# sbyrnes321/metalens

Hardware: AMD Instinct MI355X
Metric: aperture x far-field pair-evals/sec (higher is better)
Workload: dtype f64; 1 GPU; 1 mm dia NA=0.5 lens, lambda=580 nm, 4096x4096 aperture window at pitch lambda/2.2 -> 512x512 far-field directions (bins of the aperture FFT lattice x 1), fp64, on-axis x-dipole at the focus; aperture=4096, farfield=512, rings=197, centre_cells=1219855, orders=survey, pmc_key=gpus=1,aperture=4096,farfield=512,precision=f64,method=auto,zoom=1,pols=1, pmc_stale=True

## Files before the change

metalens_amd/csrc/common.h:

```cpp
#pragma once

#include <hip/hip_runtime.h>

#include <algorithm>
#include <cstdarg>
#include <cstdlib>
#include <cstdint>
#include <cstdio>
#include <cstring>
#include <string>
#include <vector>

#include "metalens_hip.h"

namespace ml {

void set_error(const char *fmt, ...);

#define ML_HIP(call)                                                                      \
    do {                                                                                  \
        hipError_t e_ = (call);                                                           \
        if (e_ != hipSuccess) {                                                           \
            ml::set_error("%s failed: %s (%s:%d)", #call, hipGetErrorString(e_), __FILE__, \
                          __LINE__);                                                      \
// ... 364 lines not shown

namespace ml {

void prof_begin(ml_ctx *ctx, int kernel, hipEvent_t *a, hipEvent_t *b, hipStream_t stream = nullptr);
void prof_end(ml_ctx *ctx, int kernel, hipEvent_t a, hipEvent_t b, hipStream_t stream = nullptr);
int prof_harvest(ml_ctx *ctx);

struct ProfScope {
    ml_ctx *ctx;
    int kernel;
    hipStream_t stream;
    hipEvent_t a = nullptr, b = nullptr;
    ProfScope(ml_ctx *c, int k, hipStream_t s = nullptr) : ctx(c), kernel(k), stream(s) {
        prof_begin(ctx, kernel, &a, &b, stream);
    }
    ~ProfScope() { prof_end(ctx, kernel, a, b, stream); }
};

int zgemm(hipStream_t stream, int M, int N, int K, const double *alpha, const double *A,
          int64_t lda, int64_t strideA, const double *B, int64_t ldb, int64_t strideB, double *C,
          int64_t ldc, int64_t strideC, int batch, int accumulate);
int zcoldot(hipStream_t stream, int n_fields, int rows, int cols, const double *alpha4,
            const double *TX, int64_t ldtx, int j0, const double *G, double *out, int accumulate);
struct FoldIO {
    int in_slabs = 1;
    int64_t in_slab_stride = 0;
    int out_t_rows = 0;
    const double *out_E = nullptr;
};
int zfold_stage1(hipStream_t stream, int M, int ny, const double *A, int64_t lda, const double *Cm,
                 const double *Sm, const double *R4, int T, int S, const double *E,
                 const double *D, double *C, int64_t ldc, int my, const int *row_first = nullptr,
                 int nxl = 1, int ksplit = 1, int64_t split_stride = 0, bool f32 = false,
                 FoldIO io = FoldIO());
int zfold_splits(int T, int ksplit);
struct ZfftCall {
    int N_eff, n_valid, M, j0, pad1, pad2;
    int jstep = 1;
    const double *in;
    int64_t in_s1, in_s2, in_es;
    int in_rb, a0, h0, a1, h1;
    const int *row_first;
    int rf_mod;
    int sub_s = 1, sub_i = 0;
    double *out;
    int64_t out_s1, out_s2, out_es;
    int out_rb;
    const double *tw1, *wk, *pj;
    const int *kbin;
    double alpha[4];
    int alpha_rb, rows, accumulate;
    int passes = 0;
    int second = 0;
};
int zfft_split(int N_eff);
bool zfft_commensurate(int n, double step, long double kappa, const double *u, int M,
                       long double tol, int *N_eff, int *j0, int *jstep);
int zfft_build_tables(hipStream_t stream, double *tw1, double *wk, double *pj, int *kbin, int M,
                      int j0, int N_eff, int c, int jstep = 1);
void zfft_choose_pads(int N_eff, int M, int j0, int *pad1, int *pad2, int jstep = 1);
int zfft_run_interleaved(hipStream_t stream, const ZfftCall &c, int s, int64_t sub_off, int stuff);
int zfft_build_interleave_tables(hipStream_t stream, double *wk, double *pj, int *kbin, int M, int j0, int Nsub,
                                 int N, int c, int first, int block, int jstep = 1);
int zfft_run(hipStream_t stream, const ZfftCall &c);
void comm_release(ml_ctx *ctx);
int fields_unmodulate(ml_ctx *ctx);
int flush_unfold(ml_ctx *ctx);
int comm_allreduce_sum(ml_ctx *ctx, double *buf, size_t count, hipStream_t stream);
int comm_reduce_scatter_sum(ml_ctx *ctx, double *buf, size_t chunk, hipStream_t stream);
int comm_allgather(ml_ctx *ctx, double *buf, size_t chunk, hipStream_t stream);
int comm_join(ml_ctx *ctx, bool host);

int nearfield_launch(ml_ctx *ctx, const ml_nearfield_params *p, int n, int nx, int ny);
int power_flush(ml_ctx *ctx);
bool plan_cache_disabled();
constexpr int POWER_GROUPS = 32;
__device__ __forceinline__ void sum_partials_group(const double *partial, int n, double *groups,
                                                   int g, int tid) {
    __shared__ double s_part[256];
    const int lo = (int)((long long)n * g / POWER_GROUPS), hi = (int)((long long)n * (g + 1) / POWER_GROUPS);
    double acc = 0.0;
    for (int k = lo + tid; k < hi; k += 256) acc += partial[k];
    __syncthreads();
    s_part[tid] = acc;
    __syncthreads();
    for (int w = 128; w > 0; w >>= 1) {
        if (tid < w) s_part[tid] += s_part[tid + w];
        __syncthreads();
    }
    if (tid == 0) groups[g] = s_part[0];
}

}
```

metalens_amd/csrc/farfield.hip:

```cpp
#include <algorithm>
#include <cmath>
#include <cstdlib>
#include <cstring>
#include <vector>

#include <cfloat>

#include "common.h"

namespace ml {

#define ML_TWO_PI_HI 6.283185307179586232e+00
#define ML_TWO_PI_LO 2.449293598294706414e-16

__global__ __launch_bounds__(256) void twiddle_kernel(double2 *out, int rows, int cols,
                                                      int sample_major, int center, double s_hi,
                                                      double s_lo, const double *u) {
    const int c = blockIdx.x * 256 + threadIdx.x;
    const int r = blockIdx.y;
    if (c >= cols) return;
    const int sample = sample_major ? r : c;
    const int dir = sample_major ? c : r;
    const double kk = (double)(sample - center);
    const double uu = u[dir];
    const double p_hi = kk * s_hi;
    const double p_lo = fma(kk, s_hi, -p_hi) + kk * s_lo;
    const double q_hi = p_hi * uu;
    const double q_lo = fma(p_hi, uu, -q_hi) + p_lo * uu;
    const double f = (q_hi - rint(q_hi)) + q_lo;
    const double a_hi = f * ML_TWO_PI_HI;
    const double ang = a_hi + (fma(f, ML_TWO_PI_HI, -a_hi) + f * ML_TWO_PI_LO);
    double sn, cs;
    sincos(ang, &sn, &cs);
    out[(size_t)r * cols + c] = make_double2(cs, -sn);
}

constexpr int MAX_PHASE_JOBS = 6;
struct PhaseJob {
    double2 *out;
    double *outc, *outs;
    int rows, cols, sample_major, block0;
    double coord0, coord_step, s_hi, s_lo;
    const double *u_hi, *u_lo;
};
struct PhaseBatch {
    PhaseJob job[MAX_PHASE_JOBS];
    int n, blocks;
};

__global__ __launch_bounds__(256) void phase_batch_kernel(const PhaseBatch b) {
    int j = 0;
    for (int k = 1; k < b.n; ++k)
        if ((int)blockIdx.x >= b.job[k].block0) j = k;
    const PhaseJob &q = b.job[j];
    const int per_row = (q.cols + 255) / 256;
    const int local = blockIdx.x - q.block0;
    const int r = local / per_row, c = (local % per_row) * 256 + threadIdx.x;
    if (c >= q.cols) return;
    const int sample = q.sample_major ? r : c;
    const int dir = q.sample_major ? c : r;
    const double kk = q.coord0 + q.coord_step * (double)sample;
// ... 591 lines not shown
    pl.wavelength = wavelength;
    pl.n_glass = n_glass;
    pl.method = method;
    ML_TRY(upload_if_changed(ctx, pl.ux, pl.h_ux, ux, mx));
    ML_TRY(upload_if_changed(ctx, pl.uy, pl.h_uy, uy, my));
    ML_TRY(pl.tw_x.reserve((size_t)mx * nx_total * 2 * sizeof(double)));
    const size_t out_elems = pair_list ? (size_t)mx : (size_t)mx * my;
    ML_TRY(pl.vectors.reserve(4 * out_elems * 2 * sizeof(double)));
    ML_TRY(pl.power.reserve(out_elems * sizeof(double)));
    ML_TRY(pl.amplitudes.reserve(2 * 2 * out_elems * 2 * sizeof(double)));
    pl.fft_y.ok = pl.fft_x.ok = false;
    if (method != ML_METHOD_GEMM && !pair_list) {
        ML_TRY(plan_fft_axis(ctx, pl.fft_y, ny, dyp, uy, my));
        ML_TRY(plan_fft_axis(ctx, pl.fft_x, nx_total, dxp, ux, mx));
    }
    pl.fold = false;
    if (!pl.fft_y.ok) ML_TRY(plan_fold(ctx, uy));
    if (!pl.fold && !pl.fft_y.ok) {
        ML_TRY(pl.tw_y.reserve((size_t)ny * my * 2 * sizeof(double)));
        ML_TRY(launch_twiddle(ctx, pl.tw_y.as<double>(), ny, my, 1, ny, dyp, wavelength, n_glass,
                              pl.uy.as<double>()));
    }
    pl.tw_x_ready = false;
    ML_TRY(plan_fold2(ctx, ux));
    pl.ready = true;
    return ML_OK;
}

static int interleave_stuff(int n_sub) {
    for (int z = 1; z <= 8; z <<= 1)
        if ((n_sub * z) % 256 == 0) return z;
    return 0;
}

static int interleave_block(const FarfieldPlan &pl, int n_ranks) {
    if (!pl.ready || pl.pair_list || !pl.fft_x.ok || n_ranks < 2) return 0;
    const int N = pl.fft_x.N_eff;
    for (int s = 8; s >= 1; s >>= 1) {
        if (N % (s * n_ranks) != 0 || pl.nx_total % (s * n_ranks) != 0) continue;
        const int stuff = interleave_stuff(N / (s * n_ranks));
        if (!stuff) continue;
        const int r3 = N / (s * n_ranks) * stuff / 256;
        if (r3 >= 1 && r3 <= 32 && r3 * s <= 32) return s;
    }
    return 0;
}

struct Shard {
    int kind = 0;
    int row0 = 0;
    int block = 0, n_ranks = 1, rank = 0;
};

static int transform_impl(ml_ctx *ctx, const Shard &sh, int accumulate) {
    ML_REQUIRE(ctx, "ctx is NULL");
    const int row0 = sh.row0, mirrored = sh.kind == 1;
    FarfieldPlan &pl = ctx->plan;
    if (!pl.ready) {
        set_error("ml_farfield_plan has not been called");
        return ML_ESTATE;
    }
    if (ctx->nx == 0) {
        set_error("no resident field set");
        return ML_ESTATE;
    }
    ML_REQUIRE(ctx->ny == pl.ny, "resident fields have ny=%d but the plan has ny=%d", ctx->ny,
               pl.ny);
    if (sh.kind == 2) {
        ML_REQUIRE(sh.block >= 1 && sh.block == interleave_block(pl, sh.n_ranks),
                   "interleaved shard: block %d is not what ml_farfield_interleave_block gives for %d ranks "
                   "on this plan (%d)", sh.block, sh.n_ranks, interleave_block(pl, sh.n_ranks));
        ML_REQUIRE(sh.rank >= 0 && sh.rank < sh.n_ranks && ctx->nx == pl.nx_total / sh.n_ranks,
                   "interleaved shard: rank %d of %d with %d resident rows of %d", sh.rank, sh.n_ranks,
                   ctx->nx, pl.nx_total);
    } else if (mirrored) {
        ML_REQUIRE(ctx->nx % 2 == 0 && row0 >= 0 && 2 * row0 + ctx->nx <= pl.nx_total,
                   "mirrored shard: %d resident rows starting at %d do not form row pairs of a "
                   "%d-row aperture", ctx->nx, row0, pl.nx_total);
        ML_REQUIRE(!pl.pair_list, "mirrored shards are for tensor grids");
    } else {
        ML_REQUIRE(row0 >= 0 && row0 + ctx->nx <= pl.nx_total,
                   "rows [%d, %d) fall outside the planned aperture of %d rows", row0,
                   row0 + ctx->nx, pl.nx_total);
    }
    ML_REQUIRE(!accumulate || pl.have_vectors, "accumulate requested but nothing to add to");
    ML_HIP(hipSetDevice(ctx->device));
    if (accumulate)
        ML_TRY(flush_unfold(ctx));
    else
        pl.unfold_pending = false;
    const int nxl = ctx->nx, ny = pl.ny, mx = pl.mx, my = pl.my;
    pl.stage1_splits = 1;
    int want_split1 = 1;
    if (pl.fold) {
        const long t128 = (long)((4 * nxl + 31) / 32) * ((pl.fold_S + 127) / 128);
        const long t64 = (long)((4 * nxl + 31) / 32) * ((pl.fold_S + 63) / 64);
        if (t128 >= 480)
            want_split1 = 1;
        else if (2 * t128 >= 480)
            want_split1 = 2;
        else
            want_split1 = (int)std::min<long>(8, std::max<long>(1, (640 + t64 - 1) / std::max<long>(t64, 1)));
        static const int forced_split = diag_int("ML_STAGE1_SPLIT", 0);
        if (forced_split > 0) want_split1 = forced_split;
        pl.stage1_splits = zfold_splits(pl.fold_T, want_split1);
    }
#ifndef ML_STAGE1_TRANSPOSED
#define ML_STAGE1_TRANSPOSED 1
#endif
    const bool g_transposed = ML_STAGE1_TRANSPOSED && pl.fft_y.ok && pl.fft_x.ok && !pl.pair_list &&
                              pl.fft_y.split == 1 && pl.fft_x.split == 1 && sh.kind != 2 &&
                              (pl.method == ML_METHOD_FFT_STREAMED ||
                               (size_t)nxl * ny * 8 + (size_t)4 * nxl * my * 16 > (size_t)96 << 20);
    static const int g_skew = diag_int("ML_G_SKEW", 8);
    const int64_t g_ld = nxl + g_skew;
    static const bool pieces_off = [] { const char *e = getenv("METALENS_HIP_PIECES"); return e && e[0] == '0'; }();
    const size_t g_bytes = g_transposed ? (size_t)4 * my * g_ld * 2 * sizeof(double)
                                        : (size_t)pl.stage1_splits * 4 * nxl * my * 2 * sizeof(double);
    const bool pieced = g_transposed && nxl <= 8192 && !pieces_off && pl.stage1_pieces.reserve(g_bytes) == ML_OK;
    if (!pieced) ML_TRY(pl.stage1.reserve(g_bytes));
    double *const g_buf = pieced ? pl.stage1_pieces.as<double>() : pl.stage1.as<double>();
    static const long fold2_min_tiles = diag_int("ML_FOLD2_MIN_TILES", 32);
    const bool whole = (row0 == 0 && nxl == pl.nx_total);
    const bool fold2_pays = (long)((4 * my + 31) / 32) * ((pl.fold2_S + 63) / 64) >= fold2_min_tiles;
    const bool fft1 = pl.fft_y.ok, fft2 = pl.fft_x.ok && !pl.pair_list;
    int trim_lo = 0, trim_hi = nxl;
    if (fft1 && fft2 && !mirrored && ctx->row_first_valid && (int)ctx->h_x_pts.size() == nxl &&
        (int)ctx->h_y_pts.size() == ny && ctx->r_outer > 0) {
        if (ctx->trim_key[0] != ctx->grid_serial || ctx->trim_key[1] != ctx->layout_serial) {
            double ymin = INFINITY;
            for (double y : ctx->h_y_pts) ymin = std::min(ymin, std::fabs(y));
            int lo = nxl, hi = 0;
            for (int i = 0; i < nxl; ++i) {
                const double x = ctx->h_x_pts[i];
                if (!(std::sqrt(x * x + ymin * ymin) > ctx->r_outer)) {
                    lo = std::min(lo, i);
                    hi = i + 1;
                }
            }
            if (lo >= hi) lo = 0, hi = std::min(nxl, 1);
            ctx->trim_rows[0] = lo;
            ctx->trim_rows[1] = hi;
            ctx->trim_key[0] = ctx->grid_serial;
            ctx->trim_key[1] = ctx->layout_serial;
        }
        static const bool no_trim = diag_int("ML_NO_ROW_TRIM", 0) != 0;
        if (!no_trim) {
            trim_lo = ctx->trim_rows[0];
            trim_hi = ctx->trim_rows[1];
        }
    }
    const int nxt = trim_hi - trim_lo;
    const bool use_fold2 = !fft2 && !pl.pair_list && pl.fold2 && fold2_pays && (mirrored || whole) && sh.kind != 2;
    static const bool no_direct = diag_int("ML_NO_GT_DIRECT", 0) != 0;
    const bool gt_direct = pl.fold && use_fold2 && !no_direct;
    FoldIO io1;
    int want_split2 = 1;
    if (gt_direct) {
        ML_TRY(stage2_tables(ctx, row0, mirrored, &want_split2));
        io1.out_t_rows = nxl;
        io1.out_E = pl.fold2_has_E ? pl.fold2_E.as<double>() : nullptr;
    }
    bool fields_premodulated = false;
    if (ctx->fields_premod_serial >= 0) {
        if (ctx->fields_premod_serial != pl.serial || !pl.fold) {
            set_error("the resident fields carry the input modulation of an earlier far-field plan "
                      "(ml_nearfield_premodulate): synthesise them again after ml_farfield_plan");
            return ML_ESTATE;
        }
        fields_premodulated = true;
    }
    const double one[4] = {1.0, 1.0, 1.0, 1.0};
    auto launch_fft1 = [&]() -> int {
        ZfftCall c;
        const int split1 = pl.fft_y.split;
        c.passes = pl.fft_y.passes;
        c.N_eff = pl.fft_y.N_eff / split1;
        c.n_valid = ny;
        c.M = my;
        c.j0 = pl.fft_y.j0;
        c.jstep = pl.fft_y.jstep;
        c.pad1 = pl.fft_y.pad1;
        c.pad2 = pl.fft_y.pad2;
        c.in = ctx->set_ptr() + (size_t)trim_lo * ny * 2;
        c.rows = 4 * nxt;
        c.in_rb = nxt;
        c.in_s1 = (int64_t)nxl * ny;
        c.in_s2 = ny;
        c.in_es = 1;
        c.a0 = 0;
        c.h0 = ny;
        c.a1 = c.h1 = 0;
        c.row_first = ctx->row_first_valid ? ctx->row_first.as<int>() + trim_lo : nullptr;
        c.rf_mod = nxt;
        c.out = g_buf + (size_t)trim_lo * my * 2;
        c.out_rb = nxt;
        c.out_s1 = (int64_t)nxl * my;
        c.out_s2 = my;
        c.out_es = 1;
        if (g_transposed) {
            c.out = g_buf + (size_t)trim_lo * 2;
            c.out_rb = nxt;
            c.out_s1 = (int64_t)my * g_ld;
            c.out_s2 = 1;
            c.out_es = g_ld;
        }
        c.tw1 = pl.fft_tw1.as<double>();
        c.wk = pl.fft_y.wk.as<double>();
        c.pj = pl.fft_y.pj.as<double>();
        c.kbin = pl.fft_y.kbin.as<int>();
        for (int k = 0; k < 4; ++k) c.alpha[k] = 1.0;
        c.alpha_rb = c.rows;
        c.accumulate = 0;
        if (split1 > 1) {
            for (int i = 0; i < split1; ++i) {
                c.sub_s = split1;
                c.sub_i = i;
                c.pj = pl.fft_y.pj.as<double>() + (size_t)i * my * 2;
                c.accumulate = i > 0;
                ML_TRY(zfft_run(ctx->stream, c));
            }
        } else {
            ML_TRY(zfft_run(ctx->stream, c));
        }
        return ML_OK;
    };
    {
        ProfScope scope(ctx, ML_K_ZGEMM_STAGE1);
        if (fft1) {
            ML_TRY(launch_fft1());
        } else if (pl.fold)
            ML_TRY(zfold_stage1(ctx->stream, 4 * nxl, ny, ctx->set_ptr(), ny,
                                pl.fold_cm.as<double>(), pl.fold_sm.as<double>(),
                                pl.fold_r4.as<double>(), pl.fold_T,
                                pl.fold_S,
                                pl.fold_has_E && !fields_premodulated ? pl.fold_E.as<double>() : nullptr,
                                pl.fold_D.as<double>(), g_buf, my, my,
                                ctx->row_first_valid ? ctx->row_first.as<int>() : nullptr, nxl,
                                want_split1, (int64_t)4 * nxl * my, ctx->gemm_f32 != 0, io1));
        else
            ML_TRY(zgemm(ctx->stream, 4 * nxl, my, ny, one, ctx->set_ptr(), ny, 0,
                         pl.tw_y.as<double>(), my, 0, g_buf, my, 0, 1, 0));
    }
    const double dA = pl.dxp * pl.dyp;
    const double alpha[4] = {-dA, dA, dA, -dA};
    auto collapse_stage1 = [&]() -> int {
        if (pl.stage1_splits > 1) {
            const size_t n = (size_t)4 * nxl * my;
            hipLaunchKernelGGL(zsum_slabs_kernel, dim3((unsigned)((n + 255) / 256)), dim3(256), 0,
                               ctx->stream, reinterpret_cast<double2 *>(g_buf), n, pl.stage1_splits);
            ML_HIP(hipGetLastError());
            pl.stage1_splits = 1;
        }
        return ML_OK;
    };
    if (sh.kind == 2) {
        ProfScope scope(ctx, ML_K_ZGEMM_STAGE2);
        ML_TRY(collapse_stage1());
// ... 14 lines not shown
        {
            ZfftCall c;
            c.N_eff = Nsub;
            c.n_valid = n_have;
            c.M = mx;
            c.j0 = pl.fft_x.j0;
            c.jstep = pl.fft_x.jstep;
            c.pad1 = pl.il_pad1;
            c.pad2 = pl.il_pad2;
            c.in = g_buf;
            c.rows = 4 * my;
            c.in_rb = my;
            c.in_s1 = (int64_t)nxl * my;
            c.in_s2 = 1;
            c.in_es = (int64_t)s * my;
            c.a0 = trim_lo;
            c.h0 = nxt;
            c.a1 = c.h1 = 0;
            c.row_first = nullptr;
            c.rf_mod = 1;
            c.out = pl.vectors.as<double>() + (size_t)3 * mx * my * 2;
            c.out_rb = my;
            c.out_s1 = -(int64_t)mx * my;
            c.out_s2 = 1;
            c.out_es = my;
            c.tw1 = pl.fft_tw1.as<double>();
            c.wk = pl.il_wk.as<double>();
            c.pj = pl.il_pj.as<double>();
            c.kbin = pl.il_kbin.as<int>();
            for (int k = 0; k < 4; ++k) c.alpha[k] = alpha[k];
            c.alpha_rb = my;
            c.accumulate = accumulate;
            ML_TRY(zfft_run_interleaved(ctx->stream, c, s, my, stuff));
        }
    } else if (fft2) {
        ProfScope scope(ctx, ML_K_ZGEMM_STAGE2);
        ML_TRY(collapse_stage1());
        ZfftCall c;
        const int split2 = pl.fft_x.split;
        c.passes = pl.fft_x.passes;
        c.N_eff = pl.fft_x.N_eff / split2;
        c.n_valid = pl.nx_total;
        c.M = mx;
        c.j0 = pl.fft_x.j0;
        c.jstep = pl.fft_x.jstep;
        c.pad1 = pl.fft_x.pad1;
        c.pad2 = pl.fft_x.pad2;
        c.in = g_buf;
        c.rows = 4 * my;
        c.in_rb = my;
        c.in_s1 = (int64_t)nxl * my;
        c.in_s2 = 1;
        c.in_es = my;
        if (g_transposed) {
            c.in_s1 = (int64_t)my * g_ld;
            c.in_s2 = g_ld;
            c.in_es = 1;
            c.second = 1;
        }
        if (mirrored) {
            c.a0 = row0;
            c.h0 = nxl / 2;
            c.a1 = pl.nx_total - row0 - nxl / 2;
            c.h1 = nxl / 2;
        } else {
            c.a0 = row0 + trim_lo;
            c.h0 = nxt;
            c.a1 = c.h1 = 0;
            c.in = g_buf + (size_t)trim_lo * c.in_es * 2;
        }
        c.row_first = nullptr;
        c.rf_mod = 1;
        c.out = pl.vectors.as<double>() + (size_t)3 * mx * my * 2;
        c.out_rb = my;
        c.out_s1 = -(int64_t)mx * my;
        c.out_s2 = 1;
        c.out_es = my;
        c.tw1 = pl.fft_tw1.as<double>();
        c.wk = pl.fft_x.wk.as<double>();
        c.pj = pl.fft_x.pj.as<double>();
        c.kbin = pl.fft_x.kbin.as<int>();
        for (int k = 0; k < 4; ++k) c.alpha[k] = alpha[k];
        c.alpha_rb = my;
        for (int i = 0; i < split2; ++i) {
            c.sub_s = split2;
            c.sub_i = i;
            c.pj = pl.fft_x.pj.as<double>() + (size_t)i * mx * 2;
            c.accumulate = i > 0 ? 1 : accumulate;
            ML_TRY(zfft_run(ctx->stream, c));
        }
    } else if (use_fold2) {
        ProfScope scope(ctx, ML_K_ZGEMM_STAGE2);
        ML_TRY(stage2_folded(ctx, row0, mirrored, accumulate, alpha, gt_direct, gt_direct,
                             want_split2));
    } else if (!pl.pair_list && mirrored) {
        ML_TRY(need_tw_x(ctx));
        ProfScope scope(ctx, ML_K_ZGEMM_STAGE2);
        ML_TRY(collapse_stage1());
        const int h = nxl / 2;
        double *slot3 = pl.vectors.as<double>() + (size_t)3 * mx * my * 2;
        for (int run = 0; run < 2; ++run) {
            const int first = run == 0 ? row0 : pl.nx_total - row0 - h;
            ML_TRY(zgemm(ctx->stream, mx, my, h, alpha, pl.tw_x.as<double>() + (size_t)first * 2,
                         pl.nx_total, 0, g_buf + (size_t)run * h * my * 2, my,
                         (int64_t)nxl * my, slot3, my, -(int64_t)mx * my, 4,
                         run == 0 ? accumulate : 1));
        }
    } else if (!pl.pair_list) {
        ML_TRY(need_tw_x(ctx));
        ProfScope scope(ctx, ML_K_ZGEMM_STAGE2);
        ML_TRY(collapse_stage1());
        double *slot3 = pl.vectors.as<double>() + (size_t)3 * mx * my * 2;
        ML_TRY(zgemm(ctx->stream, mx, my, nxl, alpha, pl.tw_x.as<double>() + (size_t)row0 * 2,
                     pl.nx_total, 0, g_buf, my, (int64_t)nxl * my, slot3, my,
                     -(int64_t)mx * my, 4, accumulate));
    } else {
        ML_TRY(need_tw_x(ctx));
        ProfScope scope(ctx, ML_K_COLDOT);
        ML_TRY(collapse_stage1());
        ML_TRY(zcoldot(ctx->stream, 4, nxl, mx, alpha, pl.tw_x.as<double>(), mx, row0,
                       g_buf, pl.vectors.as<double>(), accumulate));
    }
    pl.have_vectors = true;
    pl.amplitudes_reduced = false;
    return ML_OK;
}

static Shard block_shard(int row0, int mirrored) {
    Shard sh;
    sh.kind = mirrored ? 1 : 0;
    sh.row0 = row0;
    return sh;
}

int ml_farfield_transform_async(ml_ctx *ctx, int row0, int accumulate) {
    return transform_impl(ctx, block_shard(row0, 0), accumulate);
}
// ... 449 lines not shown
```

metalens_amd/csrc/zfft.hip:

```cpp
#include <cmath>
#include <cstdlib>
#include <map>
#include <tuple>
#include <utility>

#include "common.h"
#include "zfft_core.h"

namespace ml {

using zf::cd;

struct FftArgs {
    zf::Geo g;
    const cd *in;
    int64_t in_s1, in_s2, in_es;
    int in_rb;
    int a0, h0, a1, h1;
    const int *row_first;
    int rf_mod;
    int sub_s, sub_i;
    cd *out;
    int64_t out_s1, out_s2, out_es;
    int out_rb;
    const cd *tw1;
    const cd *wk;
    const cd *pj;
    const int *kbin;
    double alpha[4];
    int alpha_rb;
    int rows, chunk, accumulate;
};

template <int R3T>
__device__ __forceinline__ zf::Geo geo_of(const FftArgs &a) {
    zf::Geo g = a.g;
    if (R3T > 0) g.R3 = R3T;
    return g;
}

template <int R3T, bool STREAM>
__device__ __forceinline__ void load_row(const FftArgs &a, const zf::Geo &g, int row, int tid, cd *v) {
    const int NT = 16 * g.R3;
    const cd *src = a.in + (row / a.in_rb) * a.in_s1 + (row % a.in_rb) * a.in_s2;
    const int first = a.row_first ? a.row_first[row % a.rf_mod] : 0;
#pragma unroll
    for (int n2 = 0; n2 < 16; ++n2) {
        const int n = (tid + NT * n2) * a.sub_s + a.sub_i;
        int q = -1;
        if (n >= a.a0 && n < a.a0 + a.h0) q = n - a.a0;
        if (n >= a.a1 && n < a.a1 + a.h1) q = a.h0 + n - a.a1;
        if (min(n, g.n_valid - 1 - n) < first) q = -1;
        if (STREAM && q >= 0) {
            typedef double double2v __attribute__((ext_vector_type(2)));
            const double2v t = __builtin_nontemporal_load(reinterpret_cast<const double2v *>(src + q * a.in_es));
            v[n2] = zf::mk(t.x, t.y);
        } else {
            v[n2] = q >= 0 ? src[q * a.in_es] : zf::mk(0.0, 0.0);
        }
    }
}

__device__ __forceinline__ int row_of_turn(const FftArgs &a, int xcd, int idx) {
    const int row = xcd * a.chunk + idx;
    return idx < a.chunk && row < a.rows ? row : -1;
}

template <int R3T, int NTMAX, int MINW, int PASS, bool IP>
__global__ __launch_bounds__(NTMAX, MINW) void zfft_kernel(const FftArgs a) {
    extern __shared__ __align__(16) unsigned char zfft_lds_raw[];
    cd *lds = reinterpret_cast<cd *>(zfft_lds_raw);
    const zf::Geo g = geo_of<R3T>(a);
    const int NT = 16 * g.R3, tid = threadIdx.x;
    cd *s_tw = lds + zf::lds_elems(g);
    for (int e = tid; e < 256; e += NT) s_tw[(e & 15) * 16 + (e >> 4)] = a.tw1[e];
    const int n1 = tid / g.R3;
    cd tb[4];
    tb[0] = zf::mk(1.0, 0.0);
#pragma unroll
    for (int b = 1; b < 4; ++b) tb[b] = a.tw1[n1 * 16 + b];
    const int bin0 = tid, bin1 = tid + NT;
    const bool own0 = bin0 < g.M, own1 = bin1 < g.M, few = g.M <= 2 * NT;
    cd w0 = zf::mk(0, 0), p0 = w0, w1 = w0, p1 = w0;
    int k0 = 0, k1 = 0;
    if (own0) {
        w0 = a.wk[bin0];
        p0 = a.pj[bin0];
        k0 = a.kbin[bin0];
    }
    if (own1) {
        w1 = a.wk[bin1];
        p1 = a.pj[bin1];
        k1 = a.kbin[bin1];
    }
    const bool pair = own0 && own1 && ((k1 - k0) & 255) == 0;
    __syncthreads();
    const int xcd = blockIdx.x & 7, step = gridDim.x >> 3;
    int idx = blockIdx.x >> 3;
    int row = row_of_turn(a, xcd, idx);
    cd v[16], nx[16];
    if (row >= 0) load_row<R3T, PASS != 2>(a, g, row, tid, v);
    while (row >= 0) {
        const int idx_n = idx + step, row_n = row_of_turn(a, xcd, idx_n);
        const bool more = row_n >= 0;
        if (more) load_row<R3T, PASS != 2>(a, g, row_n, tid, nx);
        {
            cd ta[4];
            ta[0] = tb[0];
#pragma unroll
            for (int q = 1; q < 4; ++q) ta[q] = s_tw[(4 * q) * 16 + n1];
            zf::stage1_regs(g, tid, v, ta, tb, lds);
        }
        __syncthreads();
        zf::gather2(g, tid, v, lds);
        if (IP) {
            zf::scatter2_ip(g, tid, v, lds);
        } else {
            __syncthreads();
            zf::scatter2(g, tid, v, lds);
        }
        __syncthreads();
        cd *dst = a.out + (row / a.out_rb) * a.out_s1 + (row % a.out_rb) * a.out_s2;
        const double al = a.alpha[row / a.alpha_rb];
        if (few && pair) {
            cd xa, xb;
            if (IP)
                zf::stage3_pair_ip(g, k0, w0, w1, lds, xa, xb);
            else
                zf::stage3_pair(g, k0, w0, w1, lds, xa, xb);
            xa = zf::cmul(xa, p0);
            xb = zf::cmul(xb, p1);
            xa.x *= al;
            xa.y *= al;
            xb.x *= al;
            xb.y *= al;
            cd *da = dst + bin0 * a.out_es, *db = dst + bin1 * a.out_es;
            if (a.accumulate) {
                xa = zf::cadd(xa, *da);
                xb = zf::cadd(xb, *db);
            }
            *da = xa;
            *db = xb;
        } else if (few) {
            if (own0) {
                cd x = zf::cmul(IP ? zf::stage3_ip(g, k0, w0, lds) : zf::stage3(g, k0, w0, lds), p0);
                x.x *= al;
                x.y *= al;
                cd *d = dst + bin0 * a.out_es;
                if (a.accumulate) x = zf::cadd(x, *d);
                *d = x;
            }
            if (own1) {
                cd x = zf::cmul(IP ? zf::stage3_ip(g, k1, w1, lds) : zf::stage3(g, k1, w1, lds), p1);
                x.x *= al;
                x.y *= al;
                cd *d = dst + bin1 * a.out_es;
                if (a.accumulate) x = zf::cadd(x, *d);
                *d = x;
            }
        } else {
            for (int o = tid; o < g.M; o += NT) {
                const cd w = a.wk[o], p = a.pj[o];
                cd x = zf::cmul(IP ? zf::stage3_ip(g, a.kbin[o], w, lds) : zf::stage3(g, a.kbin[o], w, lds), p);
                x.x *= al;
                x.y *= al;
                cd *d = dst + o * a.out_es;
                if (a.accumulate) x = zf::cadd(x, *d);
                *d = x;
            }
        }
        __syncthreads();
#pragma unroll
        for (int n2 = 0; n2 < 16; ++n2) v[n2] = nx[n2];
        idx = idx_n;
        row = row_n;
    }
}

template <int R3P, int P, int NB, int MINW, int PASS>
__global__ __launch_bounds__(16 * R3P, MINW) void zfft_pass_kernel(const FftArgs a) {
    extern __shared__ __align__(16) unsigned char zfft_lds_raw[];
    cd *lds = reinterpret_cast<cd *>(zfft_lds_raw);
    zf::Geo gp = a.g, gf = a.g;
    gp.R3 = R3P;
    gf.R3 = R3P * P;
    constexpr int NT = 16 * R3P;
    const int tid = threadIdx.x;
    cd *s_tw = lds + zf::lds_elems(gp);
    for (int e = tid; e < 256; e += NT) s_tw[(e & 15) * 16 + (e >> 4)] = a.tw1[e];
    cd *s_wr = s_tw + 256;
    for (int o = tid; o < gp.M; o += NT) {
        const long long N = 256ll * R3P * P, r = ((long long)R3P * a.kbin[o]) % N;
        double sn, cs;
        sincospi(-2.0 * (double)r / (double)N, &sn, &cs);
        s_wr[o] = zf::mk(cs, sn);
    }
    const int n1 = tid / R3P, n0 = tid - n1 * R3P;
    cd tb[4];
    tb[0] = zf::mk(1.0, 0.0);
#pragma unroll
    for (int b = 1; b < 4; ++b) tb[b] = a.tw1[n1 * 16 + b];
    int kq[NB];
#pragma unroll
    for (int q = 0; q < NB; ++q) kq[q] = tid + NT * q < gp.M ? a.kbin[tid + NT * q] : 0;
    constexpr bool PAIR = (NB % 2 == 0) && (NT * (NB / 2) == 256);
    __syncthreads();
    const int xcd = blockIdx.x & 7, step = gridDim.x >> 3;
    int idx = blockIdx.x >> 3;
    int row = row_of_turn(a, xcd, idx);
    cd v[16];
    auto base_of = [&](int p) { return p * R3P + n0 + (R3P * P) * n1; };
    while (row >= 0) {
        const int idx_n = idx + step, row_n = row_of_turn(a, xcd, idx_n);
        cd acc[NB];
#pragma unroll
        for (int p = P - 1; p >= 0; --p) {
            load_row<0, PASS != 2>(a, gf, row, base_of(p), v);
            {
                cd ta[4];
                ta[0] = tb[0];
#pragma unroll
                for (int q = 1; q < 4; ++q) ta[q] = s_tw[(4 * q) * 16 + n1];
                zf::stage1_regs(gp, tid, v, ta, tb, lds);
            }
            __syncthreads();
            zf::gather2(gp, tid, v, lds);
            __syncthreads();
            zf::scatter2(gp, tid, v, lds);
// ... 350 lines not shown
    if (N < n || N < M) return false;
    long g = 256, r = N % 256;
    while (r) {
        const long t = g % r;
        g = r;
        r = t;
    }
    const long s = 256 / g, Ne = N * s;
    if (Ne > (1L << 20)) return false;
    const int R3 = (int)(Ne / 256);
    if (R3 < 1 || zfft_split((int)Ne) == 0) return false;
    const long double du_exact = 1.0L / (kappa * fabsl((long double)step) * N);
    const long jj = lrintl((long double)u[0] / du_exact);
    if (labs(jj) > (1L << 30) / s) return false;
    const long double p_max = 0.5L * n * fabsl((long double)step) + fabsl((long double)step);
    long double worst = 0;
    for (int j = 0; j < M; ++j)
        worst = fmaxl(worst, fabsl((long double)u[j] - (jj + j) * du_exact));
    if (2 * M_PIl * kappa * p_max * worst > tol) return false;
    *N_eff = (int)Ne;
    *j0 = (int)jj;
    *jstep = (int)s;
    return true;
}

int zfft_build_tables(hipStream_t stream, double *tw1, double *wk, double *pj, int *kbin, int M, int j0,
                      int N_eff, int c, int jstep) {
    const int n = M > 256 ? M : 256;
    hipLaunchKernelGGL(zfft_tables_kernel, dim3((n + 255) / 256), dim3(256), 0, stream,
                       reinterpret_cast<cd *>(tw1), reinterpret_cast<cd *>(wk),
                       reinterpret_cast<cd *>(pj), kbin, M, j0, N_eff, c, jstep);
    ML_HIP(hipGetLastError());
    return ML_OK;
}

#ifndef ML_ZFFT_IP
#define ML_ZFFT_IP 16
#endif
template <int R3T, int NTMAX, int MINW, int PASS>
static int launch_one(hipStream_t stream, const FftArgs &a, int grid, size_t lds_bytes) {
    constexpr bool IP = R3T != 0 && R3T <= ML_ZFFT_IP;
    auto kern = zfft_kernel<R3T, NTMAX, MINW, PASS, IP>;
    static bool attr_done = false;
    if (!attr_done) {
        ML_HIP(hipFuncSetAttribute(reinterpret_cast<const void *>(kern),
                                   hipFuncAttributeMaxDynamicSharedMemorySize, 160 * 1024));
        attr_done = true;
    }
    hipLaunchKernelGGL(kern, dim3(grid), dim3(16 * a.g.R3), lds_bytes, stream, a);
    ML_HIP(hipGetLastError());
    return ML_OK;
}

int zfft_run(hipStream_t stream, const ZfftCall &c) {
    FftArgs a;
    a.g.R3 = c.N_eff / 256;
    a.g.n_valid = c.n_valid;
    a.g.M = c.M;
    a.g.j0 = c.j0;
    a.g.pad1 = c.pad1;
    a.g.pad2 = c.pad2;
    a.g.ip = 0;
    a.g.jstep = c.jstep;
    a.in = reinterpret_cast<const cd *>(c.in);
    a.in_s1 = c.in_s1;
    a.in_s2 = c.in_s2;
    a.in_es = c.in_es;
    a.in_rb = c.in_rb;
    a.a0 = c.a0;
    a.h0 = c.h0;
    a.a1 = c.a1;
    a.h1 = c.h1;
    a.row_first = c.row_first;
    a.rf_mod = c.rf_mod > 0 ? c.rf_mod : 1;
    a.sub_s = c.sub_s > 0 ? c.sub_s : 1;
    a.sub_i = c.sub_i;
    a.out = reinterpret_cast<cd *>(c.out);
    a.out_s1 = c.out_s1;
    a.out_s2 = c.out_s2;
    a.out_es = c.out_es;
    a.out_rb = c.out_rb;
    a.tw1 = reinterpret_cast<const cd *>(c.tw1);
    a.wk = reinterpret_cast<const cd *>(c.wk);
    a.pj = reinterpret_cast<const cd *>(c.pj);
    a.kbin = c.kbin;
    for (int k = 0; k < 4; ++k) a.alpha[k] = c.alpha[k];
    a.alpha_rb = c.alpha_rb;
    a.rows = c.rows;
    a.accumulate = c.accumulate;
    a.chunk = (c.rows + 7) / 8;
    if (a.g.R3 <= 2) {
        const int cpw = 4 / a.g.R3;
        const size_t bytes = ((size_t)cpw * zf::lds_elems(a.g) + 256) * sizeof(cd);
        const int groups = (a.rows + cpw - 1) / cpw;
        int grid = std::min(256 * 8, (groups + 7) / 8 * 8);
        grid = std::max(grid, 8);
        if (c.in_es == 1)
            hipLaunchKernelGGL(zfft_multi_kernel<1>, dim3(grid), dim3(16 * a.g.R3 * cpw), bytes, stream, a, cpw);
        else
            hipLaunchKernelGGL(zfft_multi_kernel<2>, dim3(grid), dim3(16 * a.g.R3 * cpw), bytes, stream, a, cpw);
        ML_HIP(hipGetLastError());
        return ML_OK;
    }
    size_t lds_bytes = ((size_t)zf::lds_elems(a.g) + 256) * sizeof(cd);
    const int per_cu = (int)std::min<size_t>(8, std::max<size_t>(1, (160 * 1024) / lds_bytes));
    int grid = std::min(256 * per_cu, a.chunk * 8);
    grid = (grid + 7) / 8 * 8;
    {
        const int R3 = a.g.R3;
#ifndef ML_FFT_PASSES_R32
#define ML_FFT_PASSES_R32 2
#endif
        const int P = c.passes > 0 ? c.passes : (R3 == 32 ? ML_FFT_PASSES_R32 : 1);
        if (P > 1 && R3 % P == 0) {
            const int R3P = R3 / P, NTp = 16 * R3P, M = a.g.M;
            FftArgs ap = a;
            zfft_choose_pads(c.N_eff / P, M, c.j0, &ap.g.pad1, &ap.g.pad2, c.jstep);
            zf::Geo gp = ap.g;
            gp.R3 = R3P;
            const size_t bytes = ((size_t)zf::lds_elems(gp) + 256 + M) * sizeof(cd);
            const int per = (int)std::min<size_t>(8, std::max<size_t>(1, (160 * 1024) / bytes));
            int gridp = std::min(256 * per, a.chunk * 8);
            gridp = (gridp + 7) / 8 * 8;
            const bool p1 = c.in_es == 1;
#define ML_PASS(R, PP, NBB)                                                                   \
    if (R3P == R && P == PP && M <= NBB * NTp)                                                \
        return p1 ? (c.second ? launch_pass<R, PP, NBB, 2, 3>(stream, ap, gridp, bytes)       \
                              : launch_pass<R, PP, NBB, 2, 1>(stream, ap, gridp, bytes))      \
                  : launch_pass<R, PP, NBB, 2, 2>(stream, ap, gridp, bytes);
            ML_PASS(16, 2, 2)
            ML_PASS(32, 2, 2)
#undef ML_PASS
        }
    }
    ML_REQUIRE(a.g.R3 <= 32, "a lattice of %d samples does not fit one workgroup (%d wanted bins)", c.N_eff, c.M);
    if (a.g.R3 <= ML_ZFFT_IP && (a.g.R3 == 4 || a.g.R3 == 8 || a.g.R3 == 16 || a.g.R3 == 32)) {
        a.g.ip = 1;
        zfft_choose_pads(-c.N_eff, c.M, c.j0, &a.g.pad1, &a.g.pad2, c.jstep);
        lds_bytes = ((size_t)zf::lds_elems(a.g) + 256) * sizeof(cd);
    }
    if (c.in_es == 1 && c.second) switch (a.g.R3) {
            case 8: return launch_one<8, 128, 2, 3>(stream, a, grid, lds_bytes);
            case 16: return launch_one<16, 256, 2, 3>(stream, a, grid, lds_bytes);
            case 32: return launch_one<32, 512, 2, 3>(stream, a, grid, lds_bytes);
            default: break;
        }
    if (c.in_es == 1) switch (a.g.R3) {
            case 4: return launch_one<4, 64, 2, 1>(stream, a, grid, lds_bytes);
            case 8: return launch_one<8, 128, 2, 1>(stream, a, grid, lds_bytes);
            case 16: return launch_one<16, 256, 2, 1>(stream, a, grid, lds_bytes);
            case 32: return launch_one<32, 512, 2, 1>(stream, a, grid, lds_bytes);
            default: return launch_one<0, 512, 1, 1>(stream, a, grid, lds_bytes);
        }
    switch (a.g.R3) {
        case 4: return launch_one<4, 64, 2, 2>(stream, a, grid, lds_bytes);
        case 8: return launch_one<8, 128, 2, 2>(stream, a, grid, lds_bytes);
        case 16: return launch_one<16, 256, 2, 2>(stream, a, grid, lds_bytes);
        case 32: return launch_one<32, 512, 2, 2>(stream, a, grid, lds_bytes);
        default: return launch_one<0, 512, 1, 2>(stream, a, grid, lds_bytes);
    }
}

void zfft_choose_pads(int N_eff, int M, int j0, int *pad1, int *pad2, int jstep) {
    static std::map<std::tuple<int, int, int, int>, std::pair<int, int>> memo;
    const auto key = std::make_tuple(N_eff, M, j0, jstep);
    auto hit = memo.find(key);
    if (hit == memo.end()) {
        zf::Geo g{std::abs(N_eff) / 256, std::abs(N_eff), M, j0, 0, 0, N_eff < 0 ? 1 : 0, jstep};
        zf::choose_pads(g);
        if (memo.size() > 4096) memo.clear();
        hit = memo.emplace(key, std::make_pair(g.pad1, g.pad2)).first;
    }
    *pad1 = hit->second.first;
    *pad2 = hit->second.second;
}

}
```

metalens_amd/csrc/zfft_core.h:

```cpp
#pragma once
#include <stdint.h>

#ifdef __HIPCC__
#define ZF_HD __host__ __device__ __forceinline__
#else
#define ZF_HD inline
#include <cmath>
#endif

namespace zf {

struct alignas(16) cd {
    double x, y;
};

ZF_HD cd mk(double x, double y) {
    cd r;
    r.x = x;
    r.y = y;
    return r;
}
ZF_HD cd cadd(cd a, cd b) { return mk(a.x + b.x, a.y + b.y); }
ZF_HD cd csub(cd a, cd b) { return mk(a.x - b.x, a.y - b.y); }
ZF_HD cd cmul(cd a, cd b) {
// ... 102 lines not shown
#pragma unroll
        for (int lo = 0; lo < 4; ++lo) v[bin16(4 * hi + lo)] = cmul(v[bin16(4 * hi + lo)], w);
    }
#pragma unroll
    for (int k2 = 0; k2 < 16; ++k2) lds[ex1_addr(g, t, k2)] = v[bin16(k2)];
}
ZF_HD void gather2(const Geo &g, int u, cd *v, const cd *lds) {
    const int n0 = u % g.R3, k2 = u / g.R3;
#pragma unroll
    for (int n1 = 0; n1 < 16; ++n1) v[n1] = lds[ex1_addr(g, n0 + g.R3 * n1, k2)];
    dft16(v);
}
ZF_HD void scatter2(const Geo &g, int u, const cd *v, cd *lds) {
    const int n0 = u % g.R3, k2 = u / g.R3;
#pragma unroll
    for (int k1 = 0; k1 < 16; ++k1) lds[ex2_addr(g, n0, k1, k2)] = v[bin16(k1)];
}
ZF_HD void scatter2_ip(const Geo &g, int u, const cd *v, cd *lds) {
    const int n0 = u % g.R3, k2 = u / g.R3;
#pragma unroll
    for (int k1 = 0; k1 < 16; ++k1) lds[ex2ip_addr(g, n0, k1, k2)] = v[bin16(k1)];
}
ZF_HD cd stage3_ip(const Geo &g, int k, cd w, const cd *lds) {
    const cd *b = lds + ex2ip_addr(g, 0, (k >> 4) & 15, k & 15);
    cd x = b[g.R3 - 1];
    for (int n0 = g.R3 - 2; n0 >= 0; --n0) x = cmac(x, w, b[n0]);
    return x;
}
ZF_HD void stage3_pair_ip(const Geo &g, int k, cd wa, cd wb, const cd *lds, cd &xa, cd &xb) {
    const cd *b = lds + ex2ip_addr(g, 0, (k >> 4) & 15, k & 15);
    xa = xb = b[g.R3 - 1];
    for (int n0 = g.R3 - 2; n0 >= 0; --n0) {
        const cd t = b[n0];
        xa = cmac(xa, wa, t);
        xb = cmac(xb, wb, t);
    }
}
ZF_HD cd stage3(const Geo &g, int k, cd w, const cd *lds) {
    const int k2 = k & 15, k1 = (k >> 4) & 15;
    cd x = lds[ex2_addr(g, g.R3 - 1, k1, k2)];
    for (int n0 = g.R3 - 2; n0 >= 0; --n0) x = cmac(x, w, lds[ex2_addr(g, n0, k1, k2)]);
    return x;
}

ZF_HD void stage3_pair(const Geo &g, int k, cd wa, cd wb, const cd *lds, cd &xa, cd &xb) {
    const int k2 = k & 15, k1 = (k >> 4) & 15;
    xa = xb = lds[ex2_addr(g, g.R3 - 1, k1, k2)];
    for (int n0 = g.R3 - 2; n0 >= 0; --n0) {
        const cd t = lds[ex2_addr(g, n0, k1, k2)];
        xa = cmac(xa, wa, t);
        xb = cmac(xb, wb, t);
    }
}

}

namespace zf {

inline int lds_cycles(const int *addr, bool is_read) {
    static const int rd_groups[4][16] = {
        {0, 1, 2, 3, 12, 13, 14, 15, 20, 21, 22, 23, 24, 25, 26, 27},
        {4, 5, 6, 7, 8, 9, 10, 11, 16, 17, 18, 19, 28, 29, 30, 31},
        {32, 33, 34, 35, 44, 45, 46, 47, 52, 53, 54, 55, 56, 57, 58, 59},
        {36, 37, 38, 39, 40, 41, 42, 43, 48, 49, 50, 51, 60, 61, 62, 63}};
    int total = 0;
    const int n_groups = is_read ? 4 : 8, per = is_read ? 16 : 8, slots = is_read ? 16 : 8;
    for (int gidx = 0; gidx < n_groups; ++gidx) {
        int worst = 1;
        for (int s = 0; s < slots; ++s) {
            int seen[16], n_seen = 0;
            for (int q = 0; q < per; ++q) {
                const int lane = is_read ? rd_groups[gidx][q] : gidx * 8 + q;
                const int a = addr[lane];
                if (a < 0 || a % slots != s) continue;
                bool dup = false;
                for (int z = 0; z < n_seen; ++z) dup |= (seen[z] == a);
                if (!dup) seen[n_seen++] = a;
            }
            if (n_seen > worst) worst = n_seen;
        }
        total += worst;
    }
    return total;
}

struct LdsCost {
    long ex1_write = 0, ex1_read = 0, ex2_write = 0, ex2_read = 0, ideal_rw = 0;
};
inline LdsCost lds_cost(const Geo &g) {
    LdsCost c;
    const int NT = 16 * g.R3;
    int addr[64];
    for (int w0 = 0; w0 < NT; w0 += 64) {
        for (int s = 0; s < 16; ++s) {
            for (int l = 0; l < 64; ++l) addr[l] = w0 + l < NT ? ex1_addr(g, w0 + l, s) : -1;
            c.ex1_write += lds_cycles(addr, false);
            for (int l = 0; l < 64; ++l) {
                const int u = w0 + l;
                addr[l] = u < NT ? ex1_addr(g, u % g.R3 + g.R3 * s, u / g.R3) : -1;
            }
            c.ex1_read += lds_cycles(addr, true);
            for (int l = 0; l < 64; ++l) {
                const int u = w0 + l;
                addr[l] = u >= NT ? -1 : g.ip ? ex2ip_addr(g, u % g.R3, s, u / g.R3) : ex2_addr(g, u % g.R3, s, u / g.R3);
            }
            c.ex2_write += lds_cycles(addr, false);
            c.ideal_rw += 4 + 8;
        }
    }
    for (int o0 = 0; o0 < g.M; o0 += 64)
        for (int n0 = 0; n0 < g.R3; ++n0) {
            for (int l = 0; l < 64; ++l) {
                if (o0 + l >= g.M) {
                    addr[l] = -1;
                    continue;
                }
                const int k = bin_of(g, o0 + l);
                addr[l] = g.ip ? ex2ip_addr(g, n0, (k >> 4) & 15, k & 15) : ex2_addr(g, n0, (k >> 4) & 15, k & 15);
            }
            c.ex2_read += lds_cycles(addr, true);
        }
    return c;
}

inline void choose_pads(Geo &g) {
    long best = -1;
    int b1 = 0, b2 = 0;
    for (int p1 = 0; p1 <= 16; ++p1) {
        Geo t = g;
        t.pad1 = p1;
        t.pad2 = 0;
        const LdsCost c = lds_cost(t);
        const long cost = (c.ex1_write + c.ex1_read + (g.ip ? c.ex2_write + c.ex2_read : 0)) * 64 + p1;
        if (best < 0 || cost < best) {
            best = cost;
            b1 = p1;
        }
    }
    best = -1;
    for (int p2 = 0; p2 <= 16; ++p2) {
        Geo t = g;
        t.pad1 = b1;
        t.pad2 = p2;
        const LdsCost c = lds_cost(t);
        const long cost = (c.ex2_write + c.ex2_read) * 64 + p2;
        if (best < 0 || cost < best) {
            best = cost;
            b2 = p2;
        }
    }
    g.pad1 = b1;
    g.pad2 = b2;
}

}
```

Measured before the change: 8823000 billion pair-evals/s.

## Add tiled 8-column intermediate layout and dedicated column-pass FFT kernel

Adds a tiled layout for the stage-1 intermediate buffer, storing groups of 8 columns contiguously. The row pass writes into this layout, and a new tiles kernel performs the second-axis pass. That kernel processes 8 rows per tile with a radix-16x16 LDS decomposition, accumulating the Horner-style sum across slot rounds and using nontemporal loads. The aim is to replace the strided transposed reads of the second pass with coalesced 16-byte tile loads and better LDS reuse. The cost is a new kernel with large LDS use and occupancy 1, and it applies only under specific size conditions (my%8, mx<=512, R3 3..16).

Result: faster. 9079000 billion pair-evals/s, median of 6 (+2.9%).

```diff
diff --git a/metalens_amd/csrc/common.h b/metalens_amd/csrc/common.h
--- a/metalens_amd/csrc/common.h
+++ b/metalens_amd/csrc/common.h
@@ -440,7 +440,9 @@
     int alpha_rb, rows, accumulate;
     int passes = 0;
     int second = 0;
-};
+    int tiled_out = 0;
+};
+int zfft_run_tiles(hipStream_t stream, const ZfftCall &c);
 int zfft_split(int N_eff);
 bool zfft_commensurate(int n, double step, long double kappa, const double *u, int M,
                        long double tol, int *N_eff, int *j0, int *jstep);
diff --git a/metalens_amd/csrc/farfield.hip b/metalens_amd/csrc/farfield.hip
--- a/metalens_amd/csrc/farfield.hip
+++ b/metalens_amd/csrc/farfield.hip
@@ -7,6 +7,7 @@
 #include <cfloat>
 
 #include "common.h"
+#include "zfft_core.h"
 
 namespace ml {
 
@@ -704,6 +705,8 @@
     int block = 0, n_ranks = 1, rank = 0;
 };
 
+enum class GLayout { row_major, transposed, tiled };
+
 static int transform_impl(ml_ctx *ctx, const Shard &sh, int accumulate) {
     ML_REQUIRE(ctx, "ctx is NULL");
     const int row0 = sh.row0, mirrored = sh.kind == 1;
@@ -766,6 +769,13 @@
                                (size_t)nxl * ny * 8 + (size_t)4 * nxl * my * 16 > (size_t)96 << 20);
     static const int g_skew = diag_int("ML_G_SKEW", 8);
     const int64_t g_ld = nxl + g_skew;
+    static const bool tiles_off = diag_int("ML_G_TILED", 1) == 0;
+    const int r3y = pl.fft_y.N_eff / 256;
+    const GLayout g_layout = !g_transposed ? GLayout::row_major
+                             : (!tiles_off && my % 8 == 0 && mx <= zf::TL_NT && r3y >= 3 && r3y <= 16 &&
+                                pl.fft_y.passes <= 1 && pl.fft_x.passes <= 1)
+                                 ? GLayout::tiled
+                                 : GLayout::transposed;
     static const bool pieces_off = [] { const char *e = getenv("METALENS_HIP_PIECES"); return e && e[0] == '0'; }();
     const size_t g_bytes = g_transposed ? (size_t)4 * my * g_ld * 2 * sizeof(double)
                                         : (size_t)pl.stage1_splits * 4 * nxl * my * 2 * sizeof(double);
@@ -850,12 +860,19 @@
         c.out_s1 = (int64_t)nxl * my;
         c.out_s2 = my;
         c.out_es = 1;
-        if (g_transposed) {
+        if (g_layout == GLayout::transposed) {
             c.out = g_buf + (size_t)trim_lo * 2;
             c.out_rb = nxt;
             c.out_s1 = (int64_t)my * g_ld;
             c.out_s2 = 1;
             c.out_es = g_ld;
+        } else if (g_layout == GLayout::tiled) {
+            c.out = g_buf + (size_t)trim_lo * 8 * 2;
+            c.out_rb = nxt;
+            c.out_s1 = (int64_t)my * g_ld;
+            c.out_s2 = 8;
+            c.out_es = 8 * g_ld;
+            c.tiled_out = 1;
         }
         c.tw1 = pl.fft_tw1.as<double>();
         c.wk = pl.fft_y.wk.as<double>();
@@ -976,11 +993,16 @@
         c.in_s1 = (int64_t)nxl * my;
         c.in_s2 = 1;
         c.in_es = my;
-        if (g_transposed) {
+        if (g_layout == GLayout::transposed) {
             c.in_s1 = (int64_t)my * g_ld;
             c.in_s2 = g_ld;
             c.in_es = 1;
             c.second = 1;
+        } else if (g_layout == GLayout::tiled) {
+            c.in_s1 = (int64_t)my * g_ld;
+            c.in_s2 = 8 * g_ld;
+            c.in_rb = my / 8;
+            c.in_es = 8;
         }
         if (mirrored) {
             c.a0 = row0;
@@ -1006,7 +1028,10 @@
         c.kbin = pl.fft_x.kbin.as<int>();
         for (int k = 0; k < 4; ++k) c.alpha[k] = alpha[k];
         c.alpha_rb = my;
-        for (int i = 0; i < split2; ++i) {
+        if (g_layout == GLayout::tiled) {
+            c.accumulate = accumulate;
+            ML_TRY(zfft_run_tiles(ctx->stream, c));
+        } else for (int i = 0; i < split2; ++i) {
             c.sub_s = split2;
             c.sub_i = i;
             c.pj = pl.fft_x.pj.as<double>() + (size_t)i * mx * 2;
diff --git a/metalens_amd/csrc/zfft.hip b/metalens_amd/csrc/zfft.hip
--- a/metalens_amd/csrc/zfft.hip
+++ b/metalens_amd/csrc/zfft.hip
@@ -61,6 +61,11 @@
     }
 }
 
+template <int PASS>
+__device__ __forceinline__ int64_t out_off(const FftArgs &a, int j) {
+    return PASS == 4 ? zf::tile_off(j, a.out_es) : (int64_t)j * a.out_es;
+}
+
 __device__ __forceinline__ int row_of_turn(const FftArgs &a, int xcd, int idx) {
     const int row = xcd * a.chunk + idx;
     return idx < a.chunk && row < a.rows ? row : -1;
@@ -134,7 +139,7 @@
             xa.y *= al;
             xb.x *= al;
             xb.y *= al;
-            cd *da = dst + bin0 * a.out_es, *db = dst + bin1 * a.out_es;
+            cd *da = dst + out_off<PASS>(a, bin0), *db = dst + out_off<PASS>(a, bin1);
             if (a.accumulate) {
                 xa = zf::cadd(xa, *da);
                 xb = zf::cadd(xb, *db);
@@ -146,7 +151,7 @@
                 cd x = zf::cmul(IP ? zf::stage3_ip(g, k0, w0, lds) : zf::stage3(g, k0, w0, lds), p0);
                 x.x *= al;
                 x.y *= al;
-                cd *d = dst + bin0 * a.out_es;
+                cd *d = dst + out_off<PASS>(a, bin0);
                 if (a.accumulate) x = zf::cadd(x, *d);
                 *d = x;
             }
@@ -154,7 +159,7 @@
                 cd x = zf::cmul(IP ? zf::stage3_ip(g, k1, w1, lds) : zf::stage3(g, k1, w1, lds), p1);
                 x.x *= al;
                 x.y *= al;
-                cd *d = dst + bin1 * a.out_es;
+                cd *d = dst + out_off<PASS>(a, bin1);
                 if (a.accumulate) x = zf::cadd(x, *d);
                 *d = x;
             }
@@ -164,7 +169,7 @@
                 cd x = zf::cmul(IP ? zf::stage3_ip(g, a.kbin[o], w, lds) : zf::stage3(g, a.kbin[o], w, lds), p);
                 x.x *= al;
                 x.y *= al;
-                cd *d = dst + o * a.out_es;
+                cd *d = dst + out_off<PASS>(a, o);
                 if (a.accumulate) x = zf::cadd(x, *d);
                 *d = x;
             }
@@ -174,6 +179,91 @@
         for (int n2 = 0; n2 < 16; ++n2) v[n2] = nx[n2];
         idx = idx_n;
         row = row_n;
+    }
+}
+
+__device__ __forceinline__ void load_tile(const FftArgs &a, const cd *src, int n0, int m1, cd *v) {
+#pragma unroll
+    for (int m2 = 0; m2 < 16; ++m2) {
+        const int n = n0 + a.g.R3 * (m1 + 16 * m2);
+        int q = -1;
+        if (n0 >= 0 && n >= a.a0 && n < a.a0 + a.h0) q = n - a.a0;
+        if (n0 >= 0 && n >= a.a1 && n < a.a1 + a.h1) q = a.h0 + n - a.a1;
+        if (q >= 0) {
+            typedef double double2v __attribute__((ext_vector_type(2)));
+            const double2v t = __builtin_nontemporal_load(reinterpret_cast<const double2v *>(src + 8 * (int64_t)q));
+            v[m2] = zf::mk(t.x, t.y);
+        } else {
+            v[m2] = zf::mk(0.0, 0.0);
+        }
+    }
+}
+
+__global__ __launch_bounds__(zf::TL_NT, 1) void zfft_tiles_kernel(const FftArgs a) {
+    extern __shared__ __align__(16) unsigned char zfft_lds_raw[];
+    cd *lds = reinterpret_cast<cd *>(zfft_lds_raw);
+    constexpr int S = zf::TL_SLOTS;
+    const int R3 = a.g.R3, tid = threadIdx.x;
+    cd *s_tw = lds + S * zf::TL_SS;
+    for (int e = tid; e < 256; e += zf::TL_NT) s_tw[(e & 15) * 16 + (e >> 4)] = a.tw1[e];
+    const int m1 = zf::tl_sub(tid), col = zf::tl_col(tid), slot = zf::tl_slot(tid);
+    const bool own = tid < a.g.M;
+    cd w = zf::mk(0.0, 0.0);
+    int k = 0;
+    if (own) {
+        w = a.wk[tid];
+        k = a.kbin[tid];
+    }
+    __syncthreads();
+    const int tiles = a.rows >> 3, rounds = (R3 + S - 1) / S;
+    for (int T = blockIdx.x; T < tiles; T += gridDim.x) {
+        const cd *src = a.in + (T / a.in_rb) * a.in_s1 + (T % a.in_rb) * a.in_s2 + col;
+        cd acc[8], v[16];
+#pragma unroll
+        for (int c = 0; c < 8; ++c) acc[c] = zf::mk(0.0, 0.0);
+        load_tile(a, src, R3 - 1 - slot, m1, v);
+        for (int i = 0; i < rounds; ++i) {
+            {
+                cd ta[4], tb[4];
+                ta[0] = tb[0] = zf::mk(1.0, 0.0);
+#pragma unroll
+                for (int q = 1; q < 4; ++q) {
+                    ta[q] = s_tw[(4 * q) * 16 + m1];
+                    tb[q] = s_tw[q * 16 + m1];
+                }
+                zf::tl_phaseA(tid, v, ta, tb, lds);
+            }
+            if (i + 1 < rounds) load_tile(a, src, R3 - 1 - S * (i + 1) - slot, m1, v);
+            __syncthreads();
+            {
+                cd u[16];
+                zf::tl_phaseB(tid, u, lds);
+            }
+            __syncthreads();
+            if (own) {
+#pragma unroll 1
+                for (int s = 0; s < S; ++s) {
+                    if (R3 - 1 - S * i - s < 0) break;
+#pragma unroll
+                    for (int c = 0; c < 8; ++c) acc[c] = zf::cmac(acc[c], w, zf::tl_bin(s, c, k, lds));
+                }
+            }
+            __syncthreads();
+        }
+        if (own) {
+            const cd p = a.pj[tid];
+#pragma unroll
+            for (int c = 0; c < 8; ++c) {
+                const int row = 8 * T + c;
+                cd x = zf::cmul(acc[c], p);
+                const double al = a.alpha[row / a.alpha_rb];
+                x.x *= al;
+                x.y *= al;
+                cd *d = a.out + (row / a.out_rb) * a.out_s1 + (row % a.out_rb) * a.out_s2 + tid * a.out_es;
+                if (a.accumulate) x = zf::cadd(x, *d);
+                *d = x;
+            }
+        }
     }
 }
 
@@ -630,7 +720,7 @@
     return ML_OK;
 }
 
-int zfft_run(hipStream_t stream, const ZfftCall &c) {
+static FftArgs args_of(const ZfftCall &c) {
     FftArgs a;
     a.g.R3 = c.N_eff / 256;
     a.g.n_valid = c.n_valid;
@@ -667,6 +757,30 @@
     a.rows = c.rows;
     a.accumulate = c.accumulate;
     a.chunk = (c.rows + 7) / 8;
+    return a;
+}
+
+int zfft_run_tiles(hipStream_t stream, const ZfftCall &c) {
+    ML_REQUIRE(c.N_eff % 256 == 0 && c.M <= zf::TL_NT && c.rows % 8 == 0 && (c.sub_s <= 1) && c.in_es == 8,
+               "tiled column pass: %d samples, %d bins, %d rows", c.N_eff, c.M, c.rows);
+    const FftArgs a = args_of(c);
+    const size_t bytes = ((size_t)zf::TL_SLOTS * zf::TL_SS + 256) * sizeof(cd);
+    static bool attr_done = false;
+    if (!attr_done) {
+        ML_HIP(hipFuncSetAttribute(reinterpret_cast<const void *>(zfft_tiles_kernel),
+                                   hipFuncAttributeMaxDynamicSharedMemorySize, 160 * 1024));
+        attr_done = true;
+    }
+    const int tiles = c.rows / 8, grid = std::min(tiles, 256);
+    hipLaunchKernelGGL(zfft_tiles_kernel, dim3(grid), dim3(zf::TL_NT), bytes, stream, a);
+    ML_HIP(hipGetLastError());
+    return ML_OK;
+}
+
+int zfft_run(hipStream_t stream, const ZfftCall &c) {
+    FftArgs a = args_of(c);
+    ML_REQUIRE(!c.tiled_out || (a.g.R3 >= 3 && a.g.R3 <= 16 && c.passes <= 1 && c.in_es == 1 && !c.second),
+               "tiled row pass: %d samples", c.N_eff);
     if (a.g.R3 <= 2) {
         const int cpw = 4 / a.g.R3;
         const size_t bytes = ((size_t)cpw * zf::lds_elems(a.g) + 256) * sizeof(cd);
@@ -723,6 +837,12 @@
             case 32: return launch_one<32, 512, 2, 3>(stream, a, grid, lds_bytes);
             default: break;
         }
+    if (c.tiled_out) switch (a.g.R3) {
+            case 4: return launch_one<4, 64, 2, 4>(stream, a, grid, lds_bytes);
+            case 8: return launch_one<8, 128, 2, 4>(stream, a, grid, lds_bytes);
+            case 16: return launch_one<16, 256, 2, 4>(stream, a, grid, lds_bytes);
+            default: return launch_one<0, 512, 1, 4>(stream, a, grid, lds_bytes);
+        }
     if (c.in_es == 1) switch (a.g.R3) {
             case 4: return launch_one<4, 64, 2, 1>(stream, a, grid, lds_bytes);
             case 8: return launch_one<8, 128, 2, 1>(stream, a, grid, lds_bytes);
diff --git a/metalens_amd/csrc/zfft_core.h b/metalens_amd/csrc/zfft_core.h
--- a/metalens_amd/csrc/zfft_core.h
+++ b/metalens_amd/csrc/zfft_core.h
@@ -178,6 +178,38 @@
         xb = cmac(xb, wb, t);
     }
 }
+
+ZF_HD long long tile_off(int j, long long tile) { return (long long)(j >> 3) * tile + (j & 7); }
+constexpr int TL_NT = 512, TL_SLOTS = 4, TL_KS = 18, TL_CS = 289, TL_SS = 8 * TL_CS;
+ZF_HD int tl_addr(int s, int c, int k2, int m1) { return s * TL_SS + c * TL_CS + k2 * TL_KS + m1; }
+ZF_HD int tl_slot(int tid) { return tid >> 7; }
+ZF_HD int tl_col(int tid) { return tid & 7; }
+ZF_HD int tl_sub(int tid) { return (tid >> 3) & 15; }
+ZF_HD void tl_phaseA(int tid, cd *v, const cd *ta, const cd *tb, cd *lds) {
+    const int s = tl_slot(tid), c = tl_col(tid), m1 = tl_sub(tid);
+    dft16(v);
+#pragma unroll
+    for (int k2 = 0; k2 < 16; ++k2) {
+        const int hi = k2 >> 2, lo = k2 & 3;
+        cd a = v[bin16(k2)];
+        if (hi && lo)
+            a = cmul(a, cmul(ta[hi], tb[lo]));
+        else if (hi)
+            a = cmul(a, ta[hi]);
+        else if (lo)
+            a = cmul(a, tb[lo]);
+        lds[tl_addr(s, c, k2, m1)] = a;
+    }
+}
+ZF_HD void tl_phaseB(int tid, cd *v, cd *lds) {
+    const int s = tl_slot(tid), c = tl_col(tid), k2 = tl_sub(tid);
+#pragma unroll
+    for (int m1 = 0; m1 < 16; ++m1) v[m1] = lds[tl_addr(s, c, k2, m1)];
+    dft16(v);
+#pragma unroll
+    for (int k1 = 0; k1 < 16; ++k1) lds[tl_addr(s, c, k2, k1)] = v[bin16(k1)];
+}
+ZF_HD cd tl_bin(int s, int c, int k, const cd *lds) { return lds[tl_addr(s, c, k & 15, (k >> 4) & 15)]; }
 
 }
 
@@ -279,4 +311,33 @@
     g.pad2 = b2;
 }
 
-}
+struct TileCost {
+    long a_write = 0, b_read = 0, b_write = 0, horner = 0, ideal = 0;
+};
+inline TileCost tile_cost(int M, int j0) {
+    TileCost c;
+    int addr[64];
+    for (int w0 = 0; w0 < TL_NT; w0 += 64) {
+        for (int q = 0; q < 16; ++q) {
+            for (int l = 0; l < 64; ++l) addr[l] = tl_addr(tl_slot(w0 + l), tl_col(w0 + l), q, tl_sub(w0 + l));
+            c.a_write += lds_cycles(addr, false);
+            for (int l = 0; l < 64; ++l) addr[l] = tl_addr(tl_slot(w0 + l), tl_col(w0 + l), tl_sub(w0 + l), q);
+            c.b_read += lds_cycles(addr, true);
+            c.b_write += lds_cycles(addr, false);
+            c.ideal += 8 + 4 + 8;
+        }
+    }
+    for (int o0 = 0; o0 < M; o0 += 64)
+        for (int s = 0; s < TL_SLOTS; ++s)
+            for (int col = 0; col < 8; ++col) {
+                for (int l = 0; l < 64; ++l) {
+                    const int k = ((o0 + l + j0) % 256 + 256) % 256;
+                    addr[l] = o0 + l < M ? tl_addr(s, col, k & 15, k >> 4) : -1;
+                }
+                c.horner += lds_cycles(addr, true);
+                c.ideal += 4;
+            }
+    return c;
+}
+
+}
```
